# zeux/phyx

Measured on AMD Instinct MI355X. Metric: solver joint-visits/s (contacts/sec) on the 200k-box stack scene; solver iterations/s in extra, higher is better.
Workload: dtype f32

## Files before the change

### include/phyx_amd.h

```cpp
#ifndef PHYX_AMD_H
#define PHYX_AMD_H

#include <stddef.h>
#include <stdint.h>

#ifdef __cplusplus
extern "C" {
#endif

#define PHX_ABI_VERSION 2

typedef enum {
    PHX_OK = 0,
    PHX_ERR_INVALID = -1,
    PHX_ERR_NO_DEVICE = -2,
    PHX_ERR_HIP = -3,
    PHX_ERR_CAPACITY = -4,
    PHX_ERR_STATE = -5
} phx_status;

enum { PHX_SOLVE_SCALAR = 0, PHX_SOLVE_SSE2 = 1, PHX_SOLVE_AVX2 = 2 };
enum { PHX_ISLAND_SINGLE = 0, PHX_ISLAND_MULTIPLE = 1, PHX_ISLAND_SINGLE_SLOPPY = 2, PHX_ISLAND_MULTIPLE_SLOPPY = 3 };

typedef struct {
// ... 51 lines not shown
int phx_solver_solve_resident(phx_solver* s, const phx_body_view* bodies, int32_t body_count,
                              const void* d_contact_points, int32_t contact_point_count,
                              void* d_joints, int32_t joint_count, const phx_config* config);
int phx_bodies_to_view(int device, const void* d_bodies, int32_t body_count, const phx_body_view* out, void* stream);
int phx_view_to_bodies(int device, const phx_body_view* in, int32_t body_count, void* d_bodies, void* stream);

int phx_solver_set_body_state_bits(phx_solver* s, int32_t bits);

int phx_solver_set_shard(phx_solver* s, int32_t shard, int32_t shard_count);

int phx_solver_set_schedule_reuse(phx_solver* s, int32_t on);

int phx_solver_set_trace(phx_solver* s, int32_t on);
int phx_solver_get_island_trace(phx_solver* s, uint64_t* out, int32_t cap_groups, int32_t* groups);
int phx_solver_get_wave_trace(phx_solver* s, uint64_t* out, int32_t cap_words, int32_t* waves_per_group);

enum { PHX_XCH_PEER_ERROR = 1, PHX_XCH_SERIAL_MISMATCH = 2, PHX_XCH_TOPOLOGY_MISMATCH = 4, PHX_XCH_BAD_SEGMENT = 8 };
int    phx_solver_set_exchange_buffers(phx_solver* s, void* d_send, void* d_recv, size_t segment_capacity_bytes);
int    phx_solver_exchange_pack(phx_solver* s, const void* d_bodies, const void* d_joints, int32_t status_word, size_t* segment_bytes);
int    phx_solver_exchange_unpack(phx_solver* s, void* d_bodies, void* d_joints);
int    phx_solver_exchange_status(phx_solver* s, int32_t* status);
size_t phx_solver_exchange_segment_bytes(phx_solver* s);
int    phx_exchange_layout(const int32_t* group_bodies, const int32_t* group_slots, int32_t group_count, int32_t shard_count,
                           int32_t* group_owner, int64_t* group_offset_words, int64_t* rank_words, int64_t* segment_words);

#define PHX_COMM_ID_BYTES 128
typedef struct phx_comm phx_comm;
int  phx_comm_unique_id(void* out_id);
int  phx_comm_create(phx_comm** out, const void* unique_id, int32_t rank, int32_t nranks, int device);
void phx_comm_destroy(phx_comm* c);
// ... 183 lines not shown
```

### phyx_amd/_lib.py

```python
import ctypes as C
import os

_HERE = os.path.dirname(os.path.abspath(__file__))
LIB_PATH = os.path.join(_HERE, "libphyx_amd.so")

PHX_OK, PHX_ERR_INVALID, PHX_ERR_NO_DEVICE, PHX_ERR_HIP, PHX_ERR_CAPACITY, PHX_ERR_STATE = 0, -1, -2, -3, -4, -5


class PhxError(RuntimeError):
    def __init__(self, status, message):
        super().__init__("libphyx_amd: status %d: %s" % (status, message))
        self.status = status


class Config(C.Structure):
    _fields_ = [("solve_mode", C.c_int32), ("island_mode", C.c_int32),
                ("contact_iterations", C.c_int32), ("penetration_iterations", C.c_int32)]


class BodyView(C.Structure):
    _fields_ = [("vel", C.c_void_p), ("dvel", C.c_void_p), ("mpos", C.c_void_p)]


class SolveStats(C.Structure):
# ... 64 lines not shown
    "phx_solver_solve_resident": (C.c_int, [_vp, C.POINTER(BodyView), _i32, _vp, _i32, _vp, _i32, C.POINTER(Config)]),
    "phx_bodies_to_view": (C.c_int, [C.c_int, _vp, _i32, C.POINTER(BodyView), _vp]),
    "phx_view_to_bodies": (C.c_int, [C.c_int, C.POINTER(BodyView), _i32, _vp, _vp]),
    "phx_world_step_begin": (C.c_int, [_vp, _f32, C.POINTER(Config), C.POINTER(C.c_size_t)]),
    "phx_world_step_end": (C.c_int, [_vp, _f32]),
    "phx_world_stream": (C.c_void_p, [_vp]),
    "phx_solver_create": (C.c_int, [C.POINTER(_vp), C.c_int]),
    "phx_solver_destroy": (None, [_vp]),
    "phx_solver_solve": (C.c_int, [_vp, _vp, _i32, _vp, _i32, _vp, _i32, C.POINTER(Config)]),
    "phx_solver_solve_device": (C.c_int, [_vp, _vp, _i32, _vp, _i32, _vp, _i32, C.POINTER(Config)]),
    "phx_solver_synchronize": (C.c_int, [_vp]),
    "phx_solver_set_schedule_reuse": (C.c_int, [_vp, _i32]),
    "phx_solver_set_trace": (C.c_int, [_vp, _i32]),
    "phx_solver_get_wave_trace": (C.c_int, [_vp, _vp, _i32, C.POINTER(_i32)]),
    "phx_solver_get_island_trace": (C.c_int, [_vp, _vp, _i32, C.POINTER(_i32)]),
    "phx_solver_set_shard": (C.c_int, [_vp, _i32, _i32]),
    "phx_solver_set_body_state_bits": (C.c_int, [_vp, _i32]),
    "phx_solver_get_stats": (C.c_int, [_vp, C.POINTER(SolveStats)]),
    "phx_solver_get_schedule": (C.c_int, [_vp, _vp, _i32, _vp, _i32, C.POINTER(_i32)]),
    "phx_solver_get_groups": (C.c_int, [_vp, _vp, _i32, C.POINTER(_i32), C.POINTER(_i32)]),
    "phx_solver_get_partition": (C.c_int, [_vp, C.POINTER(_i32), C.POINTER(_i32), C.POINTER(_i32)]),
    "phx_solver_get_lanes": (C.c_int, [_vp, _vp, _vp, _i32, C.POINTER(_i32)]),
    "phx_solver_get_refreshed": (C.c_int, [_vp, _i32, _vp]),
    "phx_solver_bench": (C.c_int, [_vp, _vp, _i32, _vp, _i32, _vp, _i32, C.POINTER(Config), _i32, _i32, C.POINTER(BenchResult)]),
    "phx_solver_bench_stage": (C.c_int, [_vp, _vp, _i32, _vp, _i32, _i32]),
    "phx_solver_bench_checksum": (C.c_int, [_vp, C.POINTER(C.c_uint64)]),
    "phx_solver_bench_hooked": (C.c_int, [_vp, _vp, _i32, _vp, _i32, _vp, _i32, C.POINTER(Config), _i32, _i32, STEP_HOOK, _vp, C.POINTER(BenchResult)]),
    "phx_solver_stream": (C.c_void_p, [_vp]),
    "phx_schedule_priority": (C.c_uint64, [C.c_uint32, C.c_uint32, C.c_uint32]),
    "phx_schedule_colours": (C.c_int, [_vp, _vp, _i32, _vp, _i32, _vp, _vp, _vp, _i32, C.POINTER(_i32)]),
# ... 92 lines not shown
```

### phyx_amd/api.py

```python
import ctypes as C
import math

import numpy as np

from . import _lib
from ._lib import Config, SolveStats, BroadphaseStats, BenchResult, check

SOLVE_SCALAR, SOLVE_SSE2, SOLVE_AVX2 = 0, 1, 2
ISLAND_SINGLE, ISLAND_MULTIPLE, ISLAND_SINGLE_SLOPPY, ISLAND_MULTIPLE_SLOPPY = 0, 1, 2, 3

_vec2 = np.dtype([("x", "<f4"), ("y", "<f4")])
rigid_body_dtype = np.dtype([
    ("index", "<u4"), ("geom_size", _vec2), ("geom_xv", _vec2), ("geom_yv", _vec2), ("geom_pos", _vec2),
    ("aabb_min", _vec2), ("aabb_max", _vec2), ("velocity", _vec2), ("acceleration", _vec2),
    ("displacing_velocity", _vec2), ("angular_velocity", "<f4"), ("angular_acceleration", "<f4"),
    ("displacing_angular_velocity", "<f4"), ("inv_mass", "<f4"), ("inv_inertia", "<f4"),
    ("xv", _vec2), ("yv", _vec2), ("pos", _vec2), ("last_iteration", "<i4"), ("last_displacement_iteration", "<i4"),
])
contact_point_dtype = np.dtype([
    ("delta1", _vec2), ("delta2", _vec2), ("normal", _vec2), ("is_merged", "u1"), ("is_newly_created", "u1"),
    ("pad", "u1", (2,)), ("solver_index", "<i4"),
])
manifold_dtype = np.dtype([("body1", "<i4"), ("body2", "<i4"), ("point_count", "<i4"), ("point_index", "<i4")])
contact_joint_dtype = np.dtype([("contact_point_index", "<i4"), ("body1", "<i4"), ("body2", "<i4"),
# ... 254 lines not shown
        check(self.L.phx_solver_set_trace(self.h, (2 if waves else 1) if on else 0))

    def island_trace(self):
        n = C.c_int32(0)
        check(self.L.phx_solver_get_island_trace(self.h, None, 0, C.byref(n)))
        out = np.zeros((max(n.value, 1), 8), dtype=np.uint64)
        check(self.L.phx_solver_get_island_trace(self.h, _ptr(out), n.value, C.byref(n)))
        return out[:n.value]

    def wave_trace(self):
        n, w = C.c_int32(0), C.c_int32(0)
        check(self.L.phx_solver_get_island_trace(self.h, None, 0, C.byref(n)))
        check(self.L.phx_solver_get_wave_trace(self.h, None, 0, C.byref(w)))
        out = np.zeros((max(n.value, 1), w.value, 8), dtype=np.uint64)
        check(self.L.phx_solver_get_wave_trace(self.h, _ptr(out), out.size, C.byref(w)))
        return out[:n.value]

    def set_shard(self, shard, shard_count):
        check(self.L.phx_solver_set_shard(self.h, shard, shard_count))

    def set_comm(self, comm):
        self._comm = comm
        check(self.L.phx_solver_set_comm(self.h, comm.h if comm is not None else None))

    def set_exchange_buffers(self, send_ptr, recv_ptr, segment_capacity_bytes):
        check(self.L.phx_solver_set_exchange_buffers(self.h, C.c_void_p(int(send_ptr)), C.c_void_p(int(recv_ptr)), int(segment_capacity_bytes)))

    def exchange_pack(self, d_bodies, d_joints, status_word=0):
        seg = C.c_size_t(0)
        check(self.L.phx_solver_exchange_pack(self.h, d_bodies.ptr, d_joints.ptr, int(status_word), C.byref(seg)))
# ... 629 lines not shown
```

### phyx_amd/csrc/c_api_solver.hip

```cpp
#include "handles.h"

#include <algorithm>

extern "C" {

int phx_solver_create(phx_solver** out, int device)
{
    PHX_REQUIRE(out, "null out");
    *out = nullptr;
    PHX_TRY(phx::use_device(device));
    phx_solver* s = new (std::nothrow) phx_solver(device);
    PHX_REQUIRE(s, "out of host memory");
    int st = s->impl.init();
    if (st != PHX_OK) { delete s; return st; }
    *out = s;
    return PHX_OK;
}

void phx_solver_destroy(phx_solver* s) { delete s; }

int phx_solver_solve(phx_solver* s, phx_rigid_body* bodies, int32_t nb, const phx_contact_point* cps, int32_t ncp,
                     phx_contact_joint* joints, int32_t nj, const phx_config* cfg)
{
    PHX_REQUIRE(s && cfg, "null handle / config");
// ... 82 lines not shown
    s->impl.set_trace(on);
    return PHX_OK;
}

int phx_solver_get_island_trace(phx_solver* s, uint64_t* out, int32_t cap_groups, int32_t* groups)
{
    PHX_REQUIRE(s, "null handle");
    static_assert(sizeof(unsigned long long) == sizeof(uint64_t), "trace words");
    return s->impl.get_island_trace(reinterpret_cast<unsigned long long*>(out), cap_groups, groups);
}

int phx_solver_get_wave_trace(phx_solver* s, uint64_t* out, int32_t cap_words, int32_t* waves_per_group)
{
    PHX_REQUIRE(s, "null handle");
    return s->impl.get_wave_trace(reinterpret_cast<unsigned long long*>(out), cap_words, waves_per_group);
}

int phx_solver_get_groups(phx_solver* s, int32_t* offsets, int32_t cap, int32_t* count, int32_t* lds_count)
{
    PHX_REQUIRE(s, "null handle");
    return s->impl.get_groups(offsets, cap, count, lds_count);
}

int phx_solver_get_lanes(phx_solver* s, int32_t* leader_slot, int32_t* lane, int32_t cap, int32_t* count)
{
    PHX_REQUIRE(s, "null handle");
    return s->impl.get_lanes(leader_slot, lane, cap, count);
}

int phx_solver_get_partition(phx_solver* s, int32_t* interior_classes, int32_t* parts, int32_t* sweep_launches)
// ... 98 lines not shown
```

### phyx_amd/csrc/island_kernel.h

```cpp
#pragma once

#include "solver_kernels.h"

#include <type_traits>

namespace phx {

#define PHX_ISL_STAMP(k) do { if (TRACE && threadIdx.x == 0) iv.trace[(size_t)group * 8 + (k)] = wall_clock64(); } while (0)

template <bool HALF> struct BodyStore { using type = float4; };
template <> struct BodyStore<true> { using type = uint2; };

__device__ __forceinline__ float4 body_load(const float4* p, int i) { return p[i]; }
__device__ __forceinline__ void body_store(float4* p, int i, float4 v) { p[i] = v; }
__device__ __forceinline__ unsigned f2h_bits(float f) { return (unsigned)__half_as_ushort(__float2half_rn(f)); }
__device__ __forceinline__ float h2f_bits(unsigned h) { return __half2float(__ushort_as_half((unsigned short)h)); }
__device__ __forceinline__ float4 body_load(const uint2* p, int i)
{
    const uint2 r = p[i];
    return make_float4(h2f_bits(r.x & 0xFFFFu), h2f_bits(r.x >> 16), h2f_bits(r.y & 0xFFFFu), __int_as_float((int)(short)(r.y >> 16)));
}
__device__ __forceinline__ void body_store(uint2* p, int i, float4 v)
{
    p[i] = make_uint2(f2h_bits(v.x) | (f2h_bits(v.y) << 16), f2h_bits(v.z) | ((unsigned)(unsigned short)(short)__float_as_int(v.w) << 16));
// ... 36 lines not shown
```

### phyx_amd/csrc/island_kernel_body.h

```cpp
    using BodyT = typename BodyStore<HALF>::type;
    __shared__ BodyT imp[NB];
    __shared__ BodyT disp[NB];
    __shared__ __attribute__((aligned(16))) unsigned sw_raw[4 * NB];
    __shared__ unsigned char is_st[NB];
    __shared__ int flag_imp[3], flag_disp[3];
    __shared__ int s_commit;
    unsigned (*swi)[NB] = reinterpret_cast<unsigned (*)[NB]>(sw_raw);
    unsigned (*swd)[NB] = reinterpret_cast<unsigned (*)[NB]>(sw_raw + 2 * NB);
    float4* par = reinterpret_cast<float4*>(sw_raw);

    const int group = iv.group_list ? iv.group_list[blockIdx.x] : (int)blockIdx.x;
    if (iv.next_ctl && blockIdx.x == 0) {
        if (threadIdx.x < ISL_STAT_SLOTS) { iv.next_visits[threadIdx.x] = 0ull; iv.next_executed[2 * threadIdx.x] = 0; iv.next_executed[2 * threadIdx.x + 1] = 0; }
        if (threadIdx.x == 0) { *iv.next_ctl = 0ull; iv.next_visits[ISL_STAT_SLOTS] = ~0ull; iv.next_visits[ISL_STAT_SLOTS + 1] = 0ull; }
        if (threadIdx.x < ISL_SHARDS) iv.next_shards[threadIdx.x * ISL_SHARD_STRIDE] = 0ull;
    }
    if (iv.stamp_begin) solve_stamp_begin(v.stamps);
    if (iv.ngroups_dev && group >= *iv.ngroups_dev) return;
    if (iv.mode == ISL_COMPLETE && iv.done[group] == iv.epoch) return;
    PHX_ISL_STAMP(0);
    const unsigned long long cycles0 = TRACE ? __builtin_readcyclecounter() : 0ull;
    unsigned long long tw_work = 0, tw_bar = 0, tw_idle = 0, tw_work_big = 0; unsigned tw_nwork = 0, tw_nidle = 0, tw_nbig = 0;
    const int tid = threadIdx.x;

    constexpr int BI = (NB + T - 1) / T;
    int body_id[BI];
#pragma unroll
    for (int k = 0; k < BI; ++k) body_id[k] = tid + k * T < NB ? iv.bodies[(size_t)group * NB + tid + k * T] : -1;
    const int4 ua = iv.unit_recs[2 * ((size_t)group * T + tid)], ub = iv.unit_recs[2 * ((size_t)group * T + tid) + 1];
    const int4 d = iv.desc[group];
    const int units_word = iv.units[group];
    const int ncol = island_word_classes(units_word), nstatic = island_word_static(units_word);
    const bool live = ua.x >= 0;
#pragma unroll
    for (int k = 0; k < BI; ++k) if (tid + k * T >= d.w) body_id[k] = -1;
    const bool has2 = live && ua.y >= 0;
    const int jid0 = live ? ua.x : 0, jid1 = has2 ? ua.y : 0;
    const unsigned loc = live ? (unsigned)ub.x : 0u;
    const int col = live ? ub.y : -1;
    if (tid < 3) { flag_imp[tid] = 0; flag_disp[tid] = 0; }

    float4 rec_imp[BI], rec_disp[BI], rec_par[BI];
    float2 rec_mat[BI];
#pragma unroll
    for (int k = 0; k < BI; ++k) {
        if (body_id[k] < 0) continue;
        rec_imp[k] = bv.vel[body_id[k]]; rec_imp[k].w = __int_as_float(-1);
        rec_disp[k] = bv.dvel[body_id[k]]; rec_disp[k].w = __int_as_float(-1);
        rec_par[k] = bv.mpos[body_id[k]];
        if (MAT) rec_mat[k] = view_material<MAT>(v, body_id[k]);
    }
    IslJoint q0{}, q1{};
    float4 da0 = make_float4(0.f, 0.f, 0.f, 0.f), da1 = da0;
    int l1 = 0, l2 = 0;
    const bool verify = iv.mode == ISL_VERIFY;
    bool differs = false;
    phx_contact_joint jf{};
    if (has2) jf = joints[jid1];
    if (live) {
        const phx_contact_joint j = joints[jid0];
        const float4* cp4 = reinterpret_cast<const float4*>(&cps[clamp_index(ua.z, v.ncp)]);
        da0 = cp4[0];
        const float2 nn = *reinterpret_cast<const float2*>(cp4 + 1);
        q0.nx = nn.x; q0.ny = nn.y;
        l1 = (int)(loc & 0xFFFFu); l2 = (int)(loc >> 16);
        q0.accN = j.normal_accumulated_impulse; q0.accF = j.friction_accumulated_impulse;
        if (verify) {
            const int g1 = iv.bodies[(size_t)group * NB + l1], g2 = iv.bodies[(size_t)group * NB + l2];
            differs = j.contact_point_index != ua.z || j.body1 != g1 || j.body2 != g2;
            if (has2) differs |= jf.contact_point_index != ua.w || jf.body1 != g1 || jf.body2 != g2;
        }
    }
    if (has2) {
        const float4* cp4 = reinterpret_cast<const float4*>(&cps[clamp_index(ua.w, v.ncp)]);
        da1 = cp4[0];
        const float2 nn = *reinterpret_cast<const float2*>(cp4 + 1);
        q1.nx = nn.x; q1.ny = nn.y;
        q1.accN = jf.normal_accumulated_impulse; q1.accF = jf.friction_accumulated_impulse;
    }
#pragma unroll
    for (int k = 0; k < BI; ++k) {
        if (body_id[k] < 0) continue;
        const int i = tid + k * T;
        body_store(imp, i, rec_imp[k]);
        if (MAT) body_store(disp, i, make_float4(rec_mat[k].x, rec_mat[k].y, 0.f, 0.f));
        else body_store(disp, i, rec_disp[k]);
        par[i] = rec_par[k];
        const bool st = rec_par[k].x == 0.f && rec_par[k].y == 0.f;
        is_st[i] = st ? 1 : 0;
        differs |= st != (i < nstatic);
    }
    unsigned long long arrived_before = 0ull;
    unsigned my_arrival = 1u;
    if (verify) {
        const int any = __syncthreads_or(differs ? 1 : 0);
        my_arrival = any ? 1u + ISL_BAD : 1u;
        if (tid == 0) arrived_before = atomicAdd(&iv.shards[((int)blockIdx.x % ISL_SHARDS) * ISL_SHARD_STRIDE], (unsigned long long)my_arrival);
    } else __syncthreads();
    PHX_ISL_STAMP(1);
    float im1 = 0.f, ii1 = 0.f, im2 = 0.f, ii2 = 0.f;
    float mu = 0.3f;
    if (live) {
        const float4 p1 = par[l1], p2 = par[l2];
        if (MAT) {
            const float4 m1 = body_load(disp, l1), m2 = body_load(disp, l2);
            const float2 a = make_float2(m1.x, m1.y), b = make_float2(m2.x, m2.y);
            mu = material_mu(a, b);
            const float e = material_e(a, b);
            float4 V1 = float4{}, V2 = float4{};
            if (e != 0.f) { V1 = body_load(imp, l1); V2 = body_load(imp, l2); }
            refresh_joint<true>(q0, da0.x, da0.y, da0.z, da0.w, p1, p2, e, V1, V2);
            if (has2) refresh_joint<true>(q1, da1.x, da1.y, da1.z, da1.w, p1, p2, e, V1, V2);
        } else {
            refresh_joint(q0, da0.x, da0.y, da0.z, da0.w, p1, p2);
            if (has2) refresh_joint(q1, da1.x, da1.y, da1.z, da1.w, p1, p2);
        }
        im1 = p1.x; ii1 = p1.y; im2 = p2.x; ii2 = p2.y;
    }
    auto finite_bits = [](float x) { return (__float_as_uint(x) & 0x7f800000u) != 0x7f800000u; };
    auto joint_quiet = [&](const IslJoint& q) {
        return __float_as_uint(q.dstD) == 0u && finite_bits(q.nx) && finite_bits(q.ny) && finite_bits(q.aN1) && finite_bits(q.aN2) && finite_bits(q.cimN)
               && finite_bits(im1) && finite_bits(ii1) && finite_bits(im2) && finite_bits(ii2);
    };
    bool stirs = live && !(joint_quiet(q0) && (!has2 || joint_quiet(q1)));
#pragma unroll
    for (int k = 0; k < BI; ++k)
        if (body_id[k] >= 0) stirs |= (__float_as_uint(rec_disp[k].x) | __float_as_uint(rec_disp[k].y) | __float_as_uint(rec_disp[k].z)) != 0u;
    const bool disp_quiet = __syncthreads_or(stirs ? 1 : 0) == 0;
    if (MAT) {
#pragma unroll
        for (int k = 0; k < BI; ++k) if (body_id[k] >= 0) body_store(disp, tid + k * T, rec_disp[k]);
    }
    for (int i = tid; i < 4 * NB; i += T) sw_raw[i] = 0;
    const bool st1 = (im1 == 0.f && ii1 == 0.f), st2 = (im2 == 0.f && ii2 == 0.f);
    const bool wave_static = __any(live && (st1 || st2));
    int sm1 = st1 ? -1 : 0, sm2 = st2 ? -1 : 0;
    asm volatile("" : "+v"(sm1), "+v"(sm2));
    __syncthreads();
    PHX_ISL_STAMP(2);

    for (int c = 0; c < ncol; ++c) {
        if (col == c) {
            float4 B1 = body_load(imp, l1), B2 = body_load(imp, l2);
            prestep_joint(q0, q0.accN, q0.accF, B1, B2, im1, ii1, im2, ii2, false, false);
            if (has2) {
                if (HALF) { B1 = body_round<HALF>(B1); B2 = body_round<HALF>(B2); }
                prestep_joint(q1, q1.accN, q1.accF, B1, B2, im1, ii1, im2, ii2, false, false);
            }
            if (!st1) body_store(imp, l1, B1);
            if (!st2) body_store(imp, l2, B2);
        }
        __syncthreads();
    }

    if (verify && tid == 0) {
        const unsigned now = (unsigned)arrived_before + my_arrival;
        const unsigned shard = blockIdx.x % ISL_SHARDS, want = (iv.nexpect - shard + ISL_SHARDS - 1) / ISL_SHARDS;
        if ((now & ISL_ARRIVE_MASK) == want) atomicAdd(iv.ctl, now >= ISL_BAD ? (unsigned long long)(1u + ISL_BAD) : 1ull);
    }
    PHX_ISL_STAMP(3);
    int done_imp = 0, done_disp = (pi > 0 && disp_quiet) ? 1 : 0;
    bool imp_alive = ci > 0, disp_alive = pi > 0 && !disp_quiet;
    const int iters = ci > pi ? ci : pi;
    unsigned early_ctl = 0u;
    int it = 0, c = 0, slot = 0;
    auto peek_ctl = [&]() { if (verify && it == 3 && tid == 0 && iv.wait_polls > 0) early_ctl = (unsigned)__hip_atomic_load(iv.ctl, __ATOMIC_RELAXED, __HIP_MEMORY_SCOPE_AGENT); };
    auto next_slot = [&]() { slot = it % 3; if (tid == 0) { const int next = slot == 2 ? 0 : slot + 1; flag_imp[next] = 0; flag_disp[next] = 0; } };
    const bool wt = TRACE && iv.wave_trace;
    unsigned long long ts0 = 0ull, ts1 = 0ull; bool working = false;
    auto step_begin = [&]() { if (wt) { ts0 = __builtin_readcyclecounter(); working = __any(col == c); } };
    auto step_work_done = [&]() { if (wt) ts1 = __builtin_readcyclecounter(); };
    auto step_end = [&]() {
        if (!wt) return;
        const unsigned long long ts2 = __builtin_readcyclecounter();
        if (working) {
            if (__popcll(__ballot(col == c)) > 32) { tw_work_big += ts1 - ts0; ++tw_nbig; } else { tw_work += ts1 - ts0; ++tw_nwork; }
            tw_bar += ts2 - ts1;
        } else { tw_idle += ts2 - ts0; ++tw_nidle; }
    };
    auto half_step = [&](auto IMPC, const bool ws) {
        constexpr bool IMP = decltype(IMPC)::value;
        BodyT* const rec = IMP ? imp : disp;
        unsigned (*const sw)[NB] = IMP ? swi : swd;
        float4 B1 = body_load(rec, l1), B2 = body_load(rec, l2);
        unsigned pw1 = 0u, cw1 = 0u, pw2 = 0u, cw2 = 0u;
        if (ws) { pw1 = sw[(it - 1) & 1][l1]; cw1 = sw[it & 1][l1]; pw2 = sw[(it - 1) & 1][l2]; cw2 = sw[it & 1][l2]; }
        if (!HALF) asm volatile("" : "+v"(B1.x), "+v"(B1.y), "+v"(B1.z), "+v"(B1.w), "+v"(B2.x), "+v"(B2.y), "+v"(B2.z), "+v"(B2.w));
        if (ws) asm volatile("" : "+v"(pw1), "+v"(cw1), "+v"(pw2), "+v"(cw2));
        bool active = max(__float_as_int(B1.w), __float_as_int(B2.w)) > it - 2;
        if (ws) {
            const unsigned itu = (unsigned)it, clu = (unsigned)c;
            auto sp = [&](unsigned pw, unsigned cw) {
                return (int)(it == 0) | (int)((pw >> 16) == itu) | ((int)((cw >> 16) == itu + 1u) & (int)((0xFFFFu - (cw & 0xFFFFu)) < clu));
            };
            const int a1 = (sp(pw1, cw1) & sm1) | ((int)(__float_as_int(B1.w) > it - 2) & ~sm1);
            const int a2 = (sp(pw2, cw2) & sm2) | ((int)(__float_as_int(B2.w) > it - 2) & ~sm2);
            active = ((a1 | a2) & 1) != 0;
        }
        if (active) {
            const float4 S1 = B1, S2 = B2;
            bool prod = IMP ? impulse_productive(impulse_visit(q0, q0.accN, q0.accF, B1, B2, im1, ii1, im2, ii2, mu))
                             : displacement_productive(displacement_visit(q0, q0.accD, B1, B2, im1, ii1, im2, ii2));
            if (has2) {
                if (HALF) { B1 = body_round<HALF>(B1); B2 = body_round<HALF>(B2); }
                if (ws) {
                    B1.x = sm1 ? S1.x : B1.x; B1.y = sm1 ? S1.y : B1.y; B1.z = sm1 ? S1.z : B1.z; B1.w = sm1 ? S1.w : B1.w;
                    B2.x = sm2 ? S2.x : B2.x; B2.y = sm2 ? S2.y : B2.y; B2.z = sm2 ? S2.z : B2.z; B2.w = sm2 ? S2.w : B2.w;
                }
                prod |= IMP ? impulse_productive(impulse_visit(q1, q1.accN, q1.accF, B1, B2, im1, ii1, im2, ii2, mu))
                             : displacement_productive(displacement_visit(q1, q1.accD, B1, B2, im1, ii1, im2, ii2));
            }
            B1.w = prod ? __int_as_float(it) : B1.w; B2.w = prod ? __int_as_float(it) : B2.w;
            if (prod) {
                if (IMP) flag_imp[slot] = 1; else flag_disp[slot] = 1;
                if (ws) {
                    if (st1) atomicMax(&sw[it & 1][l1], static_word(it, c));
                    if (st2) atomicMax(&sw[it & 1][l2], static_word(it, c));
                }
            }
            if (!ws || !st1) body_store(rec, l1, B1);
            if (!ws || !st2) body_store(rec, l2, B2);
        }
    };
    const std::true_type IMPULSES{}; const std::false_type DISPLACEMENT{};
    bool hot_from_here = false;
    for (; it < iters; ++it) {
        const bool imp_on = imp_alive && it < ci, disp_on = disp_alive && it < pi;
        if (!imp_on && !disp_on) break;
        if (imp_on && !disp_on) { hot_from_here = true; break; }
        peek_ctl();
        next_slot();
        for (c = 0; c < ncol; ++c) {
            step_begin();
            if (col == c) {
                if (wave_static) {
                    if (imp_on) half_step(IMPULSES, true);
                    if (disp_on) half_step(DISPLACEMENT, true);
                } else {
                    if (imp_on) half_step(IMPULSES, false);
                    if (disp_on) half_step(DISPLACEMENT, false);
                }
            }
            step_work_done();
            __syncthreads();
            step_end();
        }
        if (imp_on) { done_imp = it + 1; imp_alive = flag_imp[slot] != 0; }
        if (disp_on) { done_disp = it + 1; disp_alive = flag_disp[slot] != 0; }
    }
    if (hot_from_here)
        for (; it < ci && imp_alive; ++it) {
            peek_ctl();
            next_slot();
            for (c = 0; c < ncol; ++c) {
                step_begin();
                if (col == c) { if (wave_static) half_step(IMPULSES, true); else half_step(IMPULSES, false); }
                step_work_done();
                __syncthreads();
                step_end();
            }
            done_imp = it + 1; imp_alive = flag_imp[slot] != 0;
        }

    PHX_ISL_STAMP(4);
    if (verify) {
        if (tid == 0) {
            const unsigned shards = iv.nexpect < (unsigned)ISL_SHARDS ? iv.nexpect : (unsigned)ISL_SHARDS;
            unsigned lo = early_ctl;
            int polls = 0;
            const bool settled = (lo & ISL_ARRIVE_MASK) >= shards || lo >= ISL_BAD;
            for (; !settled && polls < iv.wait_polls; ++polls) {
                lo = (unsigned)__hip_atomic_load(iv.ctl, __ATOMIC_RELAXED, __HIP_MEMORY_SCOPE_AGENT);
                if ((lo & ISL_ARRIVE_MASK) >= shards || lo >= ISL_BAD) break;
                __builtin_amdgcn_s_sleep(32);
            }
            s_commit = lo == shards ? 1 : 0;
            if (!settled && polls == iv.wait_polls) atomicOr(iv.ctl, ISL_TIMEOUT);
        }
        __syncthreads();
        if (!s_commit) { if (iv.stamp_end) solve_stamp_end(v.stamps); return; }
    } else if (iv.mode == ISL_GATED && *v.fingerprint != v.expected_fingerprint) { if (iv.stamp_end) solve_stamp_end(v.stamps); return; }
    if (live) {
        phx_contact_joint& out = joints[jid0];
        __builtin_nontemporal_store(q0.accN, &out.normal_accumulated_impulse);
        __builtin_nontemporal_store(q0.accF, &out.friction_accumulated_impulse);
    }
    if (has2) {
        phx_contact_joint& out = joints[jid1];
        __builtin_nontemporal_store(q1.accN, &out.normal_accumulated_impulse);
        __builtin_nontemporal_store(q1.accF, &out.friction_accumulated_impulse);
    }
#pragma unroll
    for (int k = 0; k < BI; ++k) {
        const int i = tid + k * T;
// ... 3 lines not shown
        store_nt(&bv.dvel[body_id[k]], e.x, e.y, e.z, 0.f);
    }
    if (iv.stamp_end) solve_stamp_end(v.stamps);
    if (tid == 0) {
        if (iv.mode != ISL_GATED) iv.done[group] = iv.epoch;
        const int slot = group % ISL_STAT_SLOTS;
        atomicMax(&iv.executed[2 * slot], done_imp);
        atomicMax(&iv.executed[2 * slot + 1], done_disp);
        atomicAdd(&iv.visits[slot], (unsigned long long)done_imp * (unsigned long long)d.y);
    }
    if (TRACE && iv.wave_trace && (tid & 63) == 0) {
        unsigned long long* w = iv.wave_trace + ((size_t)group * (T / 64) + (tid >> 6)) * 8;
        w[0] = tw_work; w[1] = tw_bar; w[2] = tw_idle; w[3] = ((unsigned long long)tw_nwork << 32) | tw_nidle; w[4] = tw_work_big; w[5] = tw_nbig;
        w[6] = __builtin_amdgcn_s_getreg((4 << 0) | (0 << 6) | (31 << 11));
        w[7] = __builtin_amdgcn_s_getreg((20 << 0) | (0 << 6) | (3 << 11)) & 0xF;
    }
    if (TRACE) {
        __builtin_amdgcn_s_waitcnt(0);
        PHX_ISL_STAMP(5);
        if (tid == 0) {
            iv.trace[(size_t)group * 8 + 6] = (unsigned long long)(__builtin_amdgcn_s_getreg((20 << 0) | (0 << 6) | (3 << 11)) & 0xF)
                                              | ((__builtin_readcyclecounter() - cycles0) << 4);
            iv.trace[(size_t)group * 8 + 7] = ((unsigned long long)ncol << 32) | (unsigned)done_imp;
        }
    }
```

### phyx_amd/csrc/island_view.h

```cpp
#pragma once

#include "common.h"
#include "body_view.h"

namespace phx {

struct SolverView;

enum { ISL_GATED = 0, ISL_VERIFY = 1, ISL_COMPLETE = 2 };
constexpr unsigned ISL_BAD = 1u << 20;
constexpr unsigned ISL_ARRIVE_MASK = ISL_BAD - 1u;
constexpr int ISL_SHARDS = 16, ISL_SHARD_STRIDE = 16;
constexpr unsigned long long ISL_TIMEOUT = 1ull << 40;
constexpr int ISL_WAIT_POLLS = 20000;

__host__ __device__ inline int island_units_word(int units, int classes, int nstatic) { return units | (classes << 12) | (nstatic << 20); }
__host__ __device__ inline int island_word_units(int w) { return w & 0xFFF; }
__host__ __device__ inline int island_word_classes(int w) { return (w >> 12) & 0xFF; }
__host__ __device__ inline int island_word_static(int w) { return (int)((unsigned)w >> 20); }

constexpr int ISL_T = 256, ISL_B = 768;
constexpr int ISL_T_BIG = 512, ISL_B_BIG = 1024;

struct IslandView {
    const int4* desc;
    const int* ncol;
    const int* units;
    const int4* unit_recs;
    const int* bodies;
    int* executed;
    unsigned long long* visits;
    const int* ngroups_dev;
    const int* group_list;
    int stamp_begin, stamp_end;
    unsigned long long* wave_trace;
    unsigned long long* trace;
    int mode;
    unsigned nexpect;
    unsigned long long* ctl;
    unsigned long long* shards;
    unsigned* done; unsigned epoch;
    int wait_polls;
    unsigned long long* next_ctl; int* next_executed; unsigned long long* next_visits; unsigned long long* next_shards;
};

void launch_solve_islands(hipStream_t stream, int groups, bool big_shape, bool half_state, bool trace, const SolverViewMat& v, const IslandView& iv,
                          const BodyView& bodies, phx_contact_joint* joints, const phx_contact_point* cps, int ci, int pi, bool mat = false);

int island_blocks_per_cu(bool big_shape, bool half_state, bool mat = false);

}
// ... 1 lines not shown
```

### phyx_amd/csrc/solver.h

```cpp
#pragma once

#include "common.h"
#include "body_view.h"
#include "schedule.h"
#include "comm.h"

#include <type_traits>

namespace phx {

struct SolverView {
    int nb, nj, ncp, nstatic, ncolours;
    const unsigned long long* fingerprint;
    unsigned long long expected_fingerprint;
    float4* sb_imp;
    float4* sb_disp;
    const float4* sb_par;
    float4* q0;
    float4* q1;
    float4* q2;
    int4* q3;
    float2* acc;
    float2* dd;
    float* qn;
// ... 33 lines not shown
    int prelabel_components(const float4* d_mpos, int nb, const phx_manifold* d_manifolds, int nm);
    int cancel_prelabel();
    bool prelabel_pending() const { return prelabel_pending_; }
    void build_counts(int64_t out2[2]) const { out2[0] = lite_builds_; out2[1] = full_builds_; }
    int synchronize(const std::function<int()>* while_waiting = nullptr, const MailCarrier* carrier = nullptr);
    int bodies_appended(int old_nb, int new_nb);
    int get_stats(phx_solve_stats* out);
    int get_schedule(int* order, int order_cap, int* offsets, int offsets_cap, int* ncolours);
    int set_body_state_bits(int bits);
    int set_shard(int shard, int count);
    void set_schedule_reuse(bool on) { reuse_schedule_ = on; }
    void set_materials(const float2* d_mat) { mat_ = d_mat; }
    void set_trace(int level) { trace_islands_ = level != 0; trace_waves_ = level != 1; }
    int get_island_trace(unsigned long long* out, int cap_groups, int* groups);
    int get_wave_trace(unsigned long long* out, int cap_words, int* waves_per_group);
    int get_groups(int* offsets, int cap, int* count, int* lds_count);
    int get_lanes(int* leader_slot, int* lane, int cap, int* count);
    int get_partition(int* interior_classes, int* parts, int* sweep_launches)
    {
        PHX_TRY(synchronize());
        if (interior_classes) *interior_classes = sched_.hbm_interior_classes;
        if (parts) *parts = parts_in_use() ? parts_.count : 0;
        if (sweep_launches) *sweep_launches = sweep_launches_;
        return PHX_OK;
    }
    int get_refreshed(int joint, float out30[30]);
    int bench_stage(const void* d_bodies, int nb, const void* d_joints, int nj, int steps);
    int bench(const void* d_bodies, int nb, const void* d_cps, int ncp, const void* d_joints, int nj,
              const phx_config& cfg, int warmup, int steps, phx_bench_result* out, phx_step_hook hook = nullptr, void* user = nullptr);
    int bench_checksum(unsigned long long* out);
// ... 230 lines not shown
```

### phyx_amd/csrc/solver.hip

```cpp
#include "solver.h"
#include "solver_kernels.h"

#include <algorithm>
#include <chrono>
#include <cstdlib>
#include <numeric>
#include <type_traits>

namespace phx {

static inline int grid_for(int n) { return std::max(1, std::min(div_up(n, 256), 2048)); }

constexpr int STATS_SET = 2 * ISL_STAT_SLOTS, VISITS_SET = ISL_STAT_SLOTS + 2, SHARDS_SET = ISL_SHARDS * ISL_SHARD_STRIDE;


DeviceSolver::~DeviceSolver()
{
    if (hipSetDevice(device_) != hipSuccess) return;
    if (stream_) (void)hipStreamSynchronize(stream_);
    for (hipEvent_t e : bench_events_) (void)hipEventDestroy(e);
    if (ev_fork_) (void)hipEventDestroy(ev_fork_);
    if (ev_join_) (void)hipEventDestroy(ev_join_);
    if (ev_pre_fork_) (void)hipEventDestroy(ev_pre_fork_);
    if (ev_pre_join_) (void)hipEventDestroy(ev_pre_join_);
// ... 187 lines not shown
    const SolverViewMat vm = view_mat();
    const int iters = std::max(ci, pi);
    sweep_launches_ = 0;
    if (!nj) return PHX_OK;
    const int lg = sched_.lds_groups;
    if (shard_count_ > 1) PHX_TRY(ensure_partition());
    const int mine = shard_count_ > 1 ? mine_count_ : lg;
    bool forked = false;
    if (mine) {
        IslandView iv{};
        iv.group_list = shard_count_ > 1 ? grp_mine_.p : nullptr;
        iv.ngroups_dev = spec_bins_pending_ ? bld_.bin_result.p : nullptr;
        iv.stamp_begin = iv.stamp_end = owns_hbm_group() ? 0 : 1;
        iv.desc = isl_.desc.p; iv.ncol = isl_.ncol.p; iv.units = isl_.units.p; iv.unit_recs = isl_.unit_recs.p; iv.bodies = isl_.bodies.p;
        iv.executed = isl_.stats.p + (size_t)hash_slot_ * STATS_SET; iv.visits = isl_.visits.p + (size_t)hash_slot_ * VISITS_SET;
        iv.trace = nullptr; iv.wave_trace = nullptr;
        iv.mode = mode_override >= 0 ? mode_override : isl_mode_;
        iv.nexpect = isl_nexpect_; iv.ctl = hash_.p + hash_slot_; iv.epoch = solve_epoch_;
        iv.shards = isl_.shards.p + (size_t)hash_slot_ * SHARDS_SET;
        iv.wait_polls = opt_.isl_wait_polls;
        if (iv.mode != ISL_GATED) {
            if (isl_.done.cap < (size_t)lg) {
                if (isl_.done.reserve((size_t)std::max(lg, 1)) != PHX_OK) return PHX_ERR_HIP;
                PHX_HIP(hipMemsetAsync(isl_.done.p, 0, isl_.done.cap * sizeof(unsigned), stream_));
            }
            iv.done = isl_.done.p;
        }
        if (island_clears_next_) {
            const int next = hash_slot_ ^ 1;
            iv.next_ctl = hash_.p + next; iv.next_executed = isl_.stats.p + (size_t)next * STATS_SET; iv.next_visits = isl_.visits.p + (size_t)next * VISITS_SET;
            iv.next_shards = isl_.shards.p + (size_t)next * SHARDS_SET;
            island_clears_next_ = false;
        }
        if (trace_islands_ && !mat_) {
            if (isl_.trace.reserve((size_t)std::max(lg, 1) * (8 + 128)) != PHX_OK) return PHX_ERR_HIP;
            PHX_HIP(hipMemsetAsync(isl_.trace.p, 0, (size_t)lg * (8 + 128) * sizeof(unsigned long long), stream_));
            iv.trace = isl_.trace.p;
            iv.wave_trace = trace_waves_ ? isl_.trace.p + (size_t)lg * 8 : nullptr;
        }
        const bool big = sched_.lds_lanes > ISL_T;
        forked = owns_hbm_group() && !opt_.no_side_stream && !trace_islands_ && side_stream_;
        if (forked) {
            PHX_HIP(hipEventRecord(ev_fork_, stream_));
            PHX_HIP(hipStreamWaitEvent(side_stream_, ev_fork_, 0));
        }
        launch_solve_islands(forked ? side_stream_ : stream_, mine, big, half_state_, iv.trace != nullptr, vm, iv, d_bodies, d_joints, d_cps, ci, pi, mat_ != nullptr);
        if (forked) PHX_HIP(hipEventRecord(ev_join_, side_stream_));
        ++sweep_launches_;
    }
    if (owns_hbm_group()) {
        const int ncol = (int)sched_.hbm_colour_offsets.size() - 1;
        for (int it = 0; it < iters; ++it) {
            const bool imp = it < ci, disp = it < pi;
// ... 416 lines not shown
    return PHX_OK;
}

int DeviceSolver::get_island_trace(unsigned long long* out, int cap_groups, int* groups)
{
    PHX_TRY(synchronize());
    const int lg = sched_.valid ? sched_.lds_groups : 0;
    if (groups) *groups = lg;
    if (!out) return PHX_OK;
    if (!trace_islands_ || !isl_.trace.p) { set_error("island trace is off (phx_solver_set_trace)"); return PHX_ERR_STATE; }
    if (cap_groups < lg) { set_error("island trace buffer too small"); return PHX_ERR_CAPACITY; }
    if (lg) PHX_HIP(hipMemcpy(out, isl_.trace.p, (size_t)lg * 8 * sizeof(unsigned long long), hipMemcpyDeviceToHost));
    return PHX_OK;
}

int DeviceSolver::get_wave_trace(unsigned long long* out, int cap_words, int* waves_per_group)
{
    PHX_TRY(synchronize());
    const int lg = sched_.valid ? sched_.lds_groups : 0;
    const int wpg = sched_.lds_lanes > ISL_T ? ISL_T_BIG / 64 : ISL_T / 64;
    if (waves_per_group) *waves_per_group = wpg;
    if (!out) return PHX_OK;
    if (!trace_islands_ || !isl_.trace.p) { set_error("island trace is off (phx_solver_set_trace)"); return PHX_ERR_STATE; }
    if (cap_words < lg * wpg * 8) { set_error("wave trace buffer too small"); return PHX_ERR_CAPACITY; }
    if (lg) PHX_HIP(hipMemcpy(out, isl_.trace.p + (size_t)lg * 8, (size_t)lg * wpg * 8 * sizeof(unsigned long long), hipMemcpyDeviceToHost));
    return PHX_OK;
}

int DeviceSolver::set_body_state_bits(int bits)
{
// ... 231 lines not shown
```

Before: 105.8 billion.

## Hoist island prologue loads, use dummy LDS slot for static stores, add phase trace

Adds a per-group phase-trace buffer and API for timing stages of the island kernel. It also restructures the kernel prologue: joint and contact-point loads are issued unconditionally and early so they overlap, and body loads clamp invalid ids to slot zero instead of branching. Static bodies now write to an extra dummy LDS slot instead of being skipped behind a branch, and the shared-word clear is replaced by zeroing one record per lane. The kernel now assumes NB is divisible by T, and an unconditional waitcnt added before the first barrier may serialise some memory latency.

New measurement: 108.2 billion (median of 6 runs). 1.02x the previous value.

```diff
diff --git a/include/phyx_amd.h b/include/phyx_amd.h
--- a/include/phyx_amd.h
+++ b/include/phyx_amd.h
@@ -89,6 +89,7 @@
 int phx_solver_set_trace(phx_solver* s, int32_t on);
 int phx_solver_get_island_trace(phx_solver* s, uint64_t* out, int32_t cap_groups, int32_t* groups);
 int phx_solver_get_wave_trace(phx_solver* s, uint64_t* out, int32_t cap_words, int32_t* waves_per_group);
+int phx_solver_get_phase_trace(phx_solver* s, uint64_t* out, int32_t cap_words, int32_t* words_per_group);
 
 enum { PHX_XCH_PEER_ERROR = 1, PHX_XCH_SERIAL_MISMATCH = 2, PHX_XCH_TOPOLOGY_MISMATCH = 4, PHX_XCH_BAD_SEGMENT = 8 };
 int    phx_solver_set_exchange_buffers(phx_solver* s, void* d_send, void* d_recv, size_t segment_capacity_bytes);
diff --git a/phyx_amd/_lib.py b/phyx_amd/_lib.py
--- a/phyx_amd/_lib.py
+++ b/phyx_amd/_lib.py
@@ -102,6 +102,7 @@
     "phx_solver_set_trace": (C.c_int, [_vp, _i32]),
     "phx_solver_get_wave_trace": (C.c_int, [_vp, _vp, _i32, C.POINTER(_i32)]),
     "phx_solver_get_island_trace": (C.c_int, [_vp, _vp, _i32, C.POINTER(_i32)]),
+    "phx_solver_get_phase_trace": (C.c_int, [_vp, _vp, _i32, C.POINTER(_i32)]),
     "phx_solver_set_shard": (C.c_int, [_vp, _i32, _i32]),
     "phx_solver_set_body_state_bits": (C.c_int, [_vp, _i32]),
     "phx_solver_get_stats": (C.c_int, [_vp, C.POINTER(SolveStats)]),
diff --git a/phyx_amd/api.py b/phyx_amd/api.py
--- a/phyx_amd/api.py
+++ b/phyx_amd/api.py
@@ -292,6 +292,14 @@
         check(self.L.phx_solver_get_wave_trace(self.h, None, 0, C.byref(w)))
         out = np.zeros((max(n.value, 1), w.value, 8), dtype=np.uint64)
         check(self.L.phx_solver_get_wave_trace(self.h, _ptr(out), out.size, C.byref(w)))
+        return out[:n.value]
+
+    def phase_trace(self):
+        n, w = C.c_int32(0), C.c_int32(0)
+        check(self.L.phx_solver_get_island_trace(self.h, None, 0, C.byref(n)))
+        check(self.L.phx_solver_get_phase_trace(self.h, None, 0, C.byref(w)))
+        out = np.zeros((max(n.value, 1), w.value), dtype=np.uint64)
+        check(self.L.phx_solver_get_phase_trace(self.h, _ptr(out), out.size, C.byref(w)))
         return out[:n.value]
 
     def set_shard(self, shard, shard_count):
diff --git a/phyx_amd/csrc/c_api_solver.hip b/phyx_amd/csrc/c_api_solver.hip
--- a/phyx_amd/csrc/c_api_solver.hip
+++ b/phyx_amd/csrc/c_api_solver.hip
@@ -120,6 +120,12 @@
 {
     PHX_REQUIRE(s, "null handle");
     return s->impl.get_wave_trace(reinterpret_cast<unsigned long long*>(out), cap_words, waves_per_group);
+}
+
+int phx_solver_get_phase_trace(phx_solver* s, uint64_t* out, int32_t cap_words, int32_t* words_per_group)
+{
+    PHX_REQUIRE(s, "null handle");
+    return s->impl.get_phase_trace(reinterpret_cast<unsigned long long*>(out), cap_words, words_per_group);
 }
 
 int phx_solver_get_groups(phx_solver* s, int32_t* offsets, int32_t cap, int32_t* count, int32_t* lds_count)
diff --git a/phyx_amd/csrc/island_kernel.h b/phyx_amd/csrc/island_kernel.h
--- a/phyx_amd/csrc/island_kernel.h
+++ b/phyx_amd/csrc/island_kernel.h
@@ -7,6 +7,7 @@
 namespace phx {
 
 #define PHX_ISL_STAMP(k) do { if (TRACE && threadIdx.x == 0) iv.trace[(size_t)group * 8 + (k)] = wall_clock64(); } while (0)
+#define PHX_ISL_PHASE(k) do { if (TRACE && threadIdx.x == 0 && iv.phase_trace) iv.phase_trace[(size_t)group * ISL_PHASE_WORDS + (k)] = wall_clock64(); } while (0)
 
 template <bool HALF> struct BodyStore { using type = float4; };
 template <> struct BodyStore<true> { using type = uint2; };
diff --git a/phyx_amd/csrc/island_kernel_body.h b/phyx_amd/csrc/island_kernel_body.h
--- a/phyx_amd/csrc/island_kernel_body.h
+++ b/phyx_amd/csrc/island_kernel_body.h
@@ -1,6 +1,6 @@
     using BodyT = typename BodyStore<HALF>::type;
-    __shared__ BodyT imp[NB];
-    __shared__ BodyT disp[NB];
+    __shared__ BodyT imp[NB + 1];
+    __shared__ BodyT disp[NB + 1];
     __shared__ __attribute__((aligned(16))) unsigned sw_raw[4 * NB];
     __shared__ unsigned char is_st[NB];
     __shared__ int flag_imp[3], flag_disp[3];
@@ -23,61 +23,62 @@
     unsigned long long tw_work = 0, tw_bar = 0, tw_idle = 0, tw_work_big = 0; unsigned tw_nwork = 0, tw_nidle = 0, tw_nbig = 0;
     const int tid = threadIdx.x;
 
-    constexpr int BI = (NB + T - 1) / T;
+    static_assert(NB % T == 0, "a lane owns NB / T whole body slots");
+    constexpr int BI = NB / T;
     int body_id[BI];
 #pragma unroll
-    for (int k = 0; k < BI; ++k) body_id[k] = tid + k * T < NB ? iv.bodies[(size_t)group * NB + tid + k * T] : -1;
+    for (int k = 0; k < BI; ++k) body_id[k] = iv.bodies[(size_t)group * NB + tid + k * T];
     const int4 ua = iv.unit_recs[2 * ((size_t)group * T + tid)], ub = iv.unit_recs[2 * ((size_t)group * T + tid) + 1];
     const int4 d = iv.desc[group];
     const int units_word = iv.units[group];
+    if (TRACE) { __builtin_amdgcn_s_waitcnt(0x0F70); PHX_ISL_PHASE(0); }
     const int ncol = island_word_classes(units_word), nstatic = island_word_static(units_word);
     const bool live = ua.x >= 0;
-#pragma unroll
-    for (int k = 0; k < BI; ++k) if (tid + k * T >= d.w) body_id[k] = -1;
     const bool has2 = live && ua.y >= 0;
     const int jid0 = live ? ua.x : 0, jid1 = has2 ? ua.y : 0;
     const unsigned loc = live ? (unsigned)ub.x : 0u;
     const int col = live ? ub.y : -1;
-    if (tid < 3) { flag_imp[tid] = 0; flag_disp[tid] = 0; }
-
+    const int l1 = (int)(loc & 0xFFFFu), l2 = (int)(loc >> 16);
+    const bool verify = iv.mode == ISL_VERIFY;
+    const phx_contact_joint j = joints[jid0], jf = joints[jid1];
+    const float4* const cpa = reinterpret_cast<const float4*>(&cps[clamp_index(live ? ua.z : 0, v.ncp)]);
+    const float4* const cpb = reinterpret_cast<const float4*>(&cps[clamp_index(has2 ? ua.w : 0, v.ncp)]);
+    const float4 cpa0 = cpa[0], cpb0 = cpb[0];
+    const float2 nna = *reinterpret_cast<const float2*>(cpa + 1), nnb = *reinterpret_cast<const float2*>(cpb + 1);
+#pragma unroll
+    for (int k = 0; k < BI; ++k) if (tid + k * T >= d.w) body_id[k] = -1;
     float4 rec_imp[BI], rec_disp[BI], rec_par[BI];
     float2 rec_mat[BI];
 #pragma unroll
     for (int k = 0; k < BI; ++k) {
-        if (body_id[k] < 0) continue;
-        rec_imp[k] = bv.vel[body_id[k]]; rec_imp[k].w = __int_as_float(-1);
-        rec_disp[k] = bv.dvel[body_id[k]]; rec_disp[k].w = __int_as_float(-1);
-        rec_par[k] = bv.mpos[body_id[k]];
-        if (MAT) rec_mat[k] = view_material<MAT>(v, body_id[k]);
-    }
+        const int b = body_id[k] < 0 ? 0 : body_id[k];
+        rec_imp[k] = bv.vel[b]; rec_imp[k].w = __int_as_float(-1);
+        rec_disp[k] = bv.dvel[b]; rec_disp[k].w = __int_as_float(-1);
+        rec_par[k] = bv.mpos[b];
+        if (MAT) rec_mat[k] = view_material<MAT>(v, b);
+    }
+    int g1 = 0, g2 = 0;
+    if (verify) { g1 = iv.bodies[(size_t)group * NB + l1]; g2 = iv.bodies[(size_t)group * NB + l2]; }
+    if (tid < 3) { flag_imp[tid] = 0; flag_disp[tid] = 0; }
+
     IslJoint q0{}, q1{};
     float4 da0 = make_float4(0.f, 0.f, 0.f, 0.f), da1 = da0;
-    int l1 = 0, l2 = 0;
-    const bool verify = iv.mode == ISL_VERIFY;
     bool differs = false;
-    phx_contact_joint jf{};
-    if (has2) jf = joints[jid1];
     if (live) {
-        const phx_contact_joint j = joints[jid0];
-        const float4* cp4 = reinterpret_cast<const float4*>(&cps[clamp_index(ua.z, v.ncp)]);
-        da0 = cp4[0];
-        const float2 nn = *reinterpret_cast<const float2*>(cp4 + 1);
-        q0.nx = nn.x; q0.ny = nn.y;
-        l1 = (int)(loc & 0xFFFFu); l2 = (int)(loc >> 16);
+        da0 = cpa0;
+        q0.nx = nna.x; q0.ny = nna.y;
         q0.accN = j.normal_accumulated_impulse; q0.accF = j.friction_accumulated_impulse;
         if (verify) {
-            const int g1 = iv.bodies[(size_t)group * NB + l1], g2 = iv.bodies[(size_t)group * NB + l2];
             differs = j.contact_point_index != ua.z || j.body1 != g1 || j.body2 != g2;
             if (has2) differs |= jf.contact_point_index != ua.w || jf.body1 != g1 || jf.body2 != g2;
         }
     }
     if (has2) {
-        const float4* cp4 = reinterpret_cast<const float4*>(&cps[clamp_index(ua.w, v.ncp)]);
-        da1 = cp4[0];
-        const float2 nn = *reinterpret_cast<const float2*>(cp4 + 1);
-        q1.nx = nn.x; q1.ny = nn.y;
+        da1 = cpb0;
+        q1.nx = nnb.x; q1.ny = nnb.y;
         q1.accN = jf.normal_accumulated_impulse; q1.accF = jf.friction_accumulated_impulse;
     }
+    if (TRACE) { __builtin_amdgcn_s_waitcnt(0x0F70); PHX_ISL_PHASE(1); }
 #pragma unroll
     for (int k = 0; k < BI; ++k) {
         if (body_id[k] < 0) continue;
@@ -90,12 +91,18 @@
         is_st[i] = st ? 1 : 0;
         differs |= st != (i < nstatic);
     }
+    __builtin_amdgcn_s_waitcnt(0x0F70);
     unsigned long long arrived_before = 0ull;
     unsigned my_arrival = 1u;
+    PHX_ISL_PHASE(2);
     if (verify) {
         const int any = __syncthreads_or(differs ? 1 : 0);
         my_arrival = any ? 1u + ISL_BAD : 1u;
-        if (tid == 0) arrived_before = atomicAdd(&iv.shards[((int)blockIdx.x % ISL_SHARDS) * ISL_SHARD_STRIDE], (unsigned long long)my_arrival);
+        if (tid == 0) {
+            int shard = ((int)blockIdx.x % ISL_SHARDS) * ISL_SHARD_STRIDE;
+            asm volatile("" : "+v"(shard));
+            arrived_before = atomicAdd(&iv.shards[shard], (unsigned long long)my_arrival);
+        }
     } else __syncthreads();
     PHX_ISL_STAMP(1);
     float im1 = 0.f, ii1 = 0.f, im2 = 0.f, ii2 = 0.f;
@@ -126,16 +133,19 @@
 #pragma unroll
     for (int k = 0; k < BI; ++k)
         if (body_id[k] >= 0) stirs |= (__float_as_uint(rec_disp[k].x) | __float_as_uint(rec_disp[k].y) | __float_as_uint(rec_disp[k].z)) != 0u;
+    PHX_ISL_PHASE(3);
     const bool disp_quiet = __syncthreads_or(stirs ? 1 : 0) == 0;
     if (MAT) {
 #pragma unroll
         for (int k = 0; k < BI; ++k) if (body_id[k] >= 0) body_store(disp, tid + k * T, rec_disp[k]);
     }
-    for (int i = tid; i < 4 * NB; i += T) sw_raw[i] = 0;
+#pragma unroll
+    for (int k = 0; k < BI; ++k) par[tid + k * T] = make_float4(0.f, 0.f, 0.f, 0.f);
     const bool st1 = (im1 == 0.f && ii1 == 0.f), st2 = (im2 == 0.f && ii2 == 0.f);
     const bool wave_static = __any(live && (st1 || st2));
     int sm1 = st1 ? -1 : 0, sm2 = st2 ? -1 : 0;
     asm volatile("" : "+v"(sm1), "+v"(sm2));
+    const int sl1 = st1 ? NB : l1, sl2 = st2 ? NB : l2;
     __syncthreads();
     PHX_ISL_STAMP(2);
 
@@ -147,13 +157,15 @@
                 if (HALF) { B1 = body_round<HALF>(B1); B2 = body_round<HALF>(B2); }
                 prestep_joint(q1, q1.accN, q1.accF, B1, B2, im1, ii1, im2, ii2, false, false);
             }
-            if (!st1) body_store(imp, l1, B1);
-            if (!st2) body_store(imp, l2, B2);
+            body_store(imp, sl1, B1);
+            body_store(imp, sl2, B2);
         }
         __syncthreads();
+        if (TRACE && c < 4) PHX_ISL_PHASE(4 + c);
     }
 
     if (verify && tid == 0) {
+        asm volatile("" : "+v"(arrived_before));
         const unsigned now = (unsigned)arrived_before + my_arrival;
         const unsigned shard = blockIdx.x % ISL_SHARDS, want = (iv.nexpect - shard + ISL_SHARDS - 1) / ISL_SHARDS;
         if ((now & ISL_ARRIVE_MASK) == want) atomicAdd(iv.ctl, now >= ISL_BAD ? (unsigned long long)(1u + ISL_BAD) : 1ull);
@@ -168,11 +180,15 @@
     auto next_slot = [&]() { slot = it % 3; if (tid == 0) { const int next = slot == 2 ? 0 : slot + 1; flag_imp[next] = 0; flag_disp[next] = 0; } };
     const bool wt = TRACE && iv.wave_trace;
     unsigned long long ts0 = 0ull, ts1 = 0ull; bool working = false;
-    auto step_begin = [&]() { if (wt) { ts0 = __builtin_readcyclecounter(); working = __any(col == c); } };
-    auto step_work_done = [&]() { if (wt) ts1 = __builtin_readcyclecounter(); };
-    auto step_end = [&]() {
+    unsigned tp1 = 0u, tp2 = 0u, tp3 = 0u, in_step[5] = {0u, 0u, 0u, 0u, 0u};
+    unsigned in_n = 0u;
+    auto step_begin = [&]() { if (wt) { ts0 = __builtin_readcyclecounter(); working = __any(col == c); tp3 = 0u; } };
+    auto step_work_done = [&]() { if (wt) { __builtin_amdgcn_s_waitcnt(0xC07F); ts1 = __builtin_readcyclecounter(); } };
+    auto step_end = [&](const bool hot) {
         if (!wt) return;
         const unsigned long long ts2 = __builtin_readcyclecounter();
+        if (working && hot && tp3)
+            { in_step[0] += tp1 - (unsigned)ts0; in_step[1] += tp2 - tp1; in_step[2] += tp3 - tp2; in_step[3] += (unsigned)ts1 - tp3; in_step[4] += (unsigned)(ts2 - ts1); ++in_n; }
         if (working) {
             if (__popcll(__ballot(col == c)) > 32) { tw_work_big += ts1 - ts0; ++tw_nbig; } else { tw_work += ts1 - ts0; ++tw_nwork; }
             tw_bar += ts2 - ts1;
@@ -187,6 +203,7 @@
         if (ws) { pw1 = sw[(it - 1) & 1][l1]; cw1 = sw[it & 1][l1]; pw2 = sw[(it - 1) & 1][l2]; cw2 = sw[it & 1][l2]; }
         if (!HALF) asm volatile("" : "+v"(B1.x), "+v"(B1.y), "+v"(B1.z), "+v"(B1.w), "+v"(B2.x), "+v"(B2.y), "+v"(B2.z), "+v"(B2.w));
         if (ws) asm volatile("" : "+v"(pw1), "+v"(cw1), "+v"(pw2), "+v"(cw2));
+        if (wt) { __builtin_amdgcn_s_waitcnt(0xC07F); tp1 = (unsigned)__builtin_readcyclecounter(); }
         bool active = max(__float_as_int(B1.w), __float_as_int(B2.w)) > it - 2;
         if (ws) {
             const unsigned itu = (unsigned)it, clu = (unsigned)c;
@@ -210,6 +227,7 @@
                 prod |= IMP ? impulse_productive(impulse_visit(q1, q1.accN, q1.accF, B1, B2, im1, ii1, im2, ii2, mu))
                              : displacement_productive(displacement_visit(q1, q1.accD, B1, B2, im1, ii1, im2, ii2));
             }
+            if (wt) { asm volatile("" : "+v"(B1.x), "+v"(B1.y), "+v"(B1.z), "+v"(B2.x), "+v"(B2.y), "+v"(B2.z)); tp2 = (unsigned)__builtin_readcyclecounter(); }
             B1.w = prod ? __int_as_float(it) : B1.w; B2.w = prod ? __int_as_float(it) : B2.w;
             if (prod) {
                 if (IMP) flag_imp[slot] = 1; else flag_disp[slot] = 1;
@@ -218,8 +236,9 @@
                     if (st2) atomicMax(&sw[it & 1][l2], static_word(it, c));
                 }
             }
-            if (!ws || !st1) body_store(rec, l1, B1);
-            if (!ws || !st2) body_store(rec, l2, B2);
+            body_store(rec, sl1, B1);
+            body_store(rec, sl2, B2);
+            if (wt) tp3 = (unsigned)__builtin_readcyclecounter() | 1u;
         }
     };
     const std::true_type IMPULSES{}; const std::false_type DISPLACEMENT{};
@@ -243,11 +262,13 @@
             }
             step_work_done();
             __syncthreads();
-            step_end();
+            step_end(false);
         }
         if (imp_on) { done_imp = it + 1; imp_alive = flag_imp[slot] != 0; }
         if (disp_on) { done_disp = it + 1; disp_alive = flag_disp[slot] != 0; }
-    }
+        if (TRACE && it == 0) PHX_ISL_PHASE(8);
+    }
+
     if (hot_from_here)
         for (; it < ci && imp_alive; ++it) {
             peek_ctl();
@@ -257,9 +278,10 @@
                 if (col == c) { if (wave_static) half_step(IMPULSES, true); else half_step(IMPULSES, false); }
                 step_work_done();
                 __syncthreads();
-                step_end();
+                step_end(true);
             }
             done_imp = it + 1; imp_alive = flag_imp[slot] != 0;
+            if (TRACE && it == 0) PHX_ISL_PHASE(8);
         }
 
     PHX_ISL_STAMP(4);
@@ -278,6 +300,7 @@
             if (!settled && polls == iv.wait_polls) atomicOr(iv.ctl, ISL_TIMEOUT);
         }
         __syncthreads();
+        PHX_ISL_PHASE(9);
         if (!s_commit) { if (iv.stamp_end) solve_stamp_end(v.stamps); return; }
     } else if (iv.mode == ISL_GATED && *v.fingerprint != v.expected_fingerprint) { if (iv.stamp_end) solve_stamp_end(v.stamps); return; }
     if (live) {
@@ -311,8 +334,15 @@
         w[0] = tw_work; w[1] = tw_bar; w[2] = tw_idle; w[3] = ((unsigned long long)tw_nwork << 32) | tw_nidle; w[4] = tw_work_big; w[5] = tw_nbig;
         w[6] = __builtin_amdgcn_s_getreg((4 << 0) | (0 << 6) | (31 << 11));
         w[7] = __builtin_amdgcn_s_getreg((20 << 0) | (0 << 6) | (3 << 11)) & 0xF;
+        if (iv.phase_trace) {
+            unsigned long long* p = iv.phase_trace + (size_t)group * ISL_PHASE_WORDS + 16 + (tid >> 6) * 8;
+#pragma unroll
+            for (int k = 0; k < 5; ++k) p[k] = in_step[k];
+            p[5] = in_n; p[6] = wave_static ? 1ull : 0ull;
+        }
     }
     if (TRACE) {
+        PHX_ISL_PHASE(10);
         __builtin_amdgcn_s_waitcnt(0);
         PHX_ISL_STAMP(5);
         if (tid == 0) {
diff --git a/phyx_amd/csrc/island_view.h b/phyx_amd/csrc/island_view.h
--- a/phyx_amd/csrc/island_view.h
+++ b/phyx_amd/csrc/island_view.h
@@ -19,6 +19,7 @@
 __host__ __device__ inline int island_word_classes(int w) { return (w >> 12) & 0xFF; }
 __host__ __device__ inline int island_word_static(int w) { return (int)((unsigned)w >> 20); }
 
+constexpr int ISL_PHASE_WORDS = 96;
 constexpr int ISL_T = 256, ISL_B = 768;
 constexpr int ISL_T_BIG = 512, ISL_B_BIG = 1024;
 
@@ -35,6 +36,7 @@
     int stamp_begin, stamp_end;
     unsigned long long* wave_trace;
     unsigned long long* trace;
+    unsigned long long* phase_trace;
     int mode;
     unsigned nexpect;
     unsigned long long* ctl;
diff --git a/phyx_amd/csrc/solver.h b/phyx_amd/csrc/solver.h
--- a/phyx_amd/csrc/solver.h
+++ b/phyx_amd/csrc/solver.h
@@ -71,6 +71,7 @@
     void set_trace(int level) { trace_islands_ = level != 0; trace_waves_ = level != 1; }
     int get_island_trace(unsigned long long* out, int cap_groups, int* groups);
     int get_wave_trace(unsigned long long* out, int cap_words, int* waves_per_group);
+    int get_phase_trace(unsigned long long* out, int cap_words, int* words_per_group);
     int get_groups(int* offsets, int cap, int* count, int* lds_count);
     int get_lanes(int* leader_slot, int* lane, int cap, int* count);
     int get_partition(int* interior_classes, int* parts, int* sweep_launches)
diff --git a/phyx_amd/csrc/solver.hip b/phyx_amd/csrc/solver.hip
--- a/phyx_amd/csrc/solver.hip
+++ b/phyx_amd/csrc/solver.hip
@@ -225,7 +225,7 @@
         iv.stamp_begin = iv.stamp_end = owns_hbm_group() ? 0 : 1;
         iv.desc = isl_.desc.p; iv.ncol = isl_.ncol.p; iv.units = isl_.units.p; iv.unit_recs = isl_.unit_recs.p; iv.bodies = isl_.bodies.p;
         iv.executed = isl_.stats.p + (size_t)hash_slot_ * STATS_SET; iv.visits = isl_.visits.p + (size_t)hash_slot_ * VISITS_SET;
-        iv.trace = nullptr; iv.wave_trace = nullptr;
+        iv.trace = nullptr; iv.wave_trace = nullptr; iv.phase_trace = nullptr;
         iv.mode = mode_override >= 0 ? mode_override : isl_mode_;
         iv.nexpect = isl_nexpect_; iv.ctl = hash_.p + hash_slot_; iv.epoch = solve_epoch_;
         iv.shards = isl_.shards.p + (size_t)hash_slot_ * SHARDS_SET;
@@ -244,10 +244,11 @@
             island_clears_next_ = false;
         }
         if (trace_islands_ && !mat_) {
-            if (isl_.trace.reserve((size_t)std::max(lg, 1) * (8 + 128)) != PHX_OK) return PHX_ERR_HIP;
-            PHX_HIP(hipMemsetAsync(isl_.trace.p, 0, (size_t)lg * (8 + 128) * sizeof(unsigned long long), stream_));
+            if (isl_.trace.reserve((size_t)std::max(lg, 1) * (8 + 128 + ISL_PHASE_WORDS)) != PHX_OK) return PHX_ERR_HIP;
+            PHX_HIP(hipMemsetAsync(isl_.trace.p, 0, (size_t)lg * (8 + 128 + ISL_PHASE_WORDS) * sizeof(unsigned long long), stream_));
             iv.trace = isl_.trace.p;
             iv.wave_trace = trace_waves_ ? isl_.trace.p + (size_t)lg * 8 : nullptr;
+            iv.phase_trace = isl_.trace.p + (size_t)lg * (8 + 128);
         }
         const bool big = sched_.lds_lanes > ISL_T;
         forked = owns_hbm_group() && !opt_.no_side_stream && !trace_islands_ && side_stream_;
@@ -694,6 +695,18 @@
     return PHX_OK;
 }
 
+int DeviceSolver::get_phase_trace(unsigned long long* out, int cap_words, int* words_per_group)
+{
+    PHX_TRY(synchronize());
+    const int lg = sched_.valid ? sched_.lds_groups : 0;
+    if (words_per_group) *words_per_group = ISL_PHASE_WORDS;
+    if (!out) return PHX_OK;
+    if (!trace_islands_ || !isl_.trace.p) { set_error("island trace is off (phx_solver_set_trace)"); return PHX_ERR_STATE; }
+    if (cap_words < lg * ISL_PHASE_WORDS) { set_error("phase trace buffer too small"); return PHX_ERR_CAPACITY; }
+    if (lg) PHX_HIP(hipMemcpy(out, isl_.trace.p + (size_t)lg * (8 + 128), (size_t)lg * ISL_PHASE_WORDS * sizeof(unsigned long long), hipMemcpyDeviceToHost));
+    return PHX_OK;
+}
+
 int DeviceSolver::get_wave_trace(unsigned long long* out, int cap_words, int* waves_per_group)
 {
     PHX_TRY(synchronize());
```
